# shibatch/rectdetect

Hardware: AMD Instinct MI355X
Metric: 1920x1080 frames/sec (higher is better)
Workload: dtype u8/i32/f32 (bit-exact integer + IEEE f32 stencil path)

## Files before the change

### rectdetect_amd/csrc/rd_k_front.hip

```cpp
#include <stdlib.h>
#include "rd_device.h"
#include "rd_kernels.h"
#include "rectdetect_hip.h"

#define RD_LUT_ATTR __device__
#include "rd_luts.h"

namespace {

using namespace rd;
using namespace rdpix;

struct P3 { float *p[3]; };
struct P3c { const float *p[3]; };
struct SrcZ { const uint8_t *p[RD_ZB_MAX]; };

inline int cdiv(int a, int b) { return (a + b - 1) / b; }
inline dim3 grid2(int iw, int ih) { return dim3(cdiv(iw, 64), cdiv(ih, 4)); }
const dim3 block2(64, 4);
inline int grid1(int n) { int g = cdiv(n, 256); return g < 1 ? 1 : g; }

__device__ __forceinline__ int lerp_lut(const unsigned short *t, int c) { return t[c >> 8] * (256 - (c & 255)) + t[(c >> 8) + 1] * (c & 255); }

__device__ __forceinline__ uint32_t plab_of(const unsigned short *s_s2l, const unsigned short *s_cf, const unsigned short *s_cf2, int b, int g, int r) {
// ... 218 lines not shown
    int pb, pg, pr;
    if (!is_yuv(FMT)) {
      const int i = 4 * RW * sr + rdpix::bpp(FMT) * sx, c[3] = { byte(i), byte(i + 1), byte(i + 2) };
      pb = c[rb_swapped(FMT) ? 2 : 0]; pg = c[1]; pr = c[rb_swapped(FMT) ? 0 : 2];
    } else if (FMT == RD_PIX_NV12) yuv_bgr(byte(8 * sr + sx), byte(16 + 2 * j), byte(17 + 2 * j), pb, pg, pr);
    else yuv_bgr(byte(8 * sr + sx), byte(16 + j), byte(20 + j), pb, pg, pr);
    b += pb; g += pg; r += pr;
  }
  b >>= 2; g >>= 2; r >>= 2;
}

template <int FMT>
__global__ __launch_bounds__(256) void k_pix2plab_half_t(uint32_t *__restrict__ out, P3 dst, PixZ src, int iw, int ih, size_t zs) {
  const int z = blockIdx.z;
  const uint8_t *__restrict__ p0 = src.p[0][z], *__restrict__ p1 = src.p[1][z], *__restrict__ p2 = src.p[2][z];
  RD_ZSHIFT(zs, out, dst.p[0], dst.p[1], dst.p[2]);
  __shared__ unsigned short s_s2l[RD_LUT_S2L_N], s_cf[RD_LUT_CF_N], s_cf2[RD_LUT_CF_N];
  __shared__ unsigned short tile[3][64][66];
  const int tid = rd_ty() * 64 + threadIdx.x;
  const int x0 = blockIdx.x * 64, y0 = blockIdx.y * 64;
  const int cx = (tid & 15) * 4, r0 = tid >> 4;
  const int x = x0 + cx, m = min(iw - x, 4);
  uint32_t w[4][HalfW<FMT>::n] = {};
#pragma unroll
  for (int k = 0; k < 4; k++) {
    const int y = y0 + r0 + 16 * k;
    if (m > 0 && y < ih) pix_load_half<FMT>(w[k], p0, p1, p2, src.pitch, x, y, m, src.wide != 0);
  }
  for (int i = tid; i < RD_LUT_S2L_N; i += 256) s_s2l[i] = rd_lut_s2l[i];
  for (int i = tid; i < RD_LUT_CF_N; i += 256) { s_cf[i] = rd_lut_cfunc[i]; s_cf2[i] = rd_lut_cfunc2[i]; }
  __syncthreads();
#pragma unroll
  for (int k = 0; k < 4; k++) {
    const int r = r0 + 16 * k, y = y0 + r;
    if (m <= 0 || y >= ih) continue;
    uint32_t v[4];
#pragma unroll
    for (int j = 0; j < 4; j++) {
      int b, g, rr;
      pix_bgr_half<FMT>(w[k], j, b, g, rr);
      v[j] = plab_of(s_s2l, s_cf, s_cf2, b, g, rr);
      tile[0][r][cx + j] = (unsigned short)(v[j] & 4095u); tile[1][r][cx + j] = (unsigned short)((v[j] >> 12) & 1023u); tile[2][r][cx + j] = (unsigned short)((v[j] >> 22) & 1023u);
    }
    uint32_t *o = out + (size_t)y * iw + x;
    if (m == 4 && (iw & 3) == 0) *(uint4 *)o = make_uint4(v[0], v[1], v[2], v[3]);
    else for (int j = 0; j < m; j++) o[j] = v[j];
  }
  __syncthreads();
  for (int r = rd_ty(); r < 64; r += 4) {
    const int ox = y0 + threadIdx.x, oy = x0 + r;
    if (ox < ih && oy < iw)
      for (int k = 0; k < 3; k++) ((unsigned short *)dst.p[k])[(size_t)oy * ih + ox] = tile[k][threadIdx.x][r];
  }
}

template <typename LD, typename ST> __device__ __forceinline__ void ew4(int n, LD ld, ST st) {
  const int stride = gridDim.x * blockDim.x;
  int i = blockIdx.x * blockDim.x + threadIdx.x;
  for (; i + 3 * stride < n; i += 4 * stride) {
    const auto v0 = ld(i), v1 = ld(i + stride), v2 = ld(i + 2 * stride), v3 = ld(i + 3 * stride);
    st(i, v0); st(i + stride, v1); st(i + 2 * stride, v2); st(i + 3 * stride, v3);
  }
  for (; i < n; i += stride) st(i, ld(i));
}

__global__ void k_unpack_plab(float *__restrict__ L, float *__restrict__ a, float *__restrict__ b, const uint32_t *__restrict__ in, int n) {
  for (int i = blockIdx.x * blockDim.x + threadIdx.x; i < n; i += gridDim.x * blockDim.x) {
    float l, aa, bb;
    unpack_lab(in[i], l, aa, bb);
    L[i] = l; a[i] = aa; b[i] = bb;
  }
}

__global__ void k_pack_plab(uint32_t *__restrict__ out, const float *__restrict__ L, const float *__restrict__ a, const float *__restrict__ b, int n) {
  ew4(n, [=](int i) { return make_float3(L[i], a[i], b[i]); }, [=](int i, float3 v) { out[i] = pack_lab(v.x, v.y, v.z); });
}

template <int MODE>
__global__ __launch_bounds__(256) void k_transpose(P3 dst, P3c src, P3c fwd, P3c bwd, const uint32_t *__restrict__ plab, int np, int W, int H, const int *only_if) {
  if (only_if && *only_if == 0) return;
  __shared__ float tile[3][64][65];
  const int x0 = blockIdx.x * 64, y0 = blockIdx.y * 64;
  for (int r = rd_ty(); r < 64; r += 4) {
    const int x = x0 + threadIdx.x, y = y0 + r;
    if (x < W && y < H) {
      const size_t i = (size_t)y * W + x;
      if (MODE == 1) {
        float l, a, b;
        unpack_lab(plab[i], l, a, b);
        tile[0][r][threadIdx.x] = l; tile[1][r][threadIdx.x] = a; tile[2][r][threadIdx.x] = b;
      } else if (MODE == 2) {
        for (int k = 0; k < np; k++) tile[k][r][threadIdx.x] = bwd.p[k][i] + fwd.p[k][i] - src.p[k][i] * 0.3989422804f;
      } else {
        for (int k = 0; k < np; k++) tile[k][r][threadIdx.x] = src.p[k][i];
      }
    }
  }
  __syncthreads();
  for (int r = rd_ty(); r < 64; r += 4) {
    const int ox = y0 + threadIdx.x, oy = x0 + r;
    if (ox < H && oy < W)
      for (int k = 0; k < np; k++) dst.p[k][(size_t)oy * H + ox] = tile[k][threadIdx.x][r];
  }
}

#define IIR_C0 0.3989422804f
#define IIR_C1 0.1414542400f
#define IIR_C2 -0.0030406818f
#define IIR_C3 -0.0041116157f
#define IIR_C4 0.0006696623f
#define IIR_C5 0.0000498707f
#define IIR_C6 -0.0000449761f
#define IIR_C7 -0.0000051528f
#define IIR_C8 0.2519574622f
#define IIR_C9 -0.0098627835f
#define IIR_C10 -0.0067013653f
#define IIR_C11 0.0012572396f
#define IIR_C12 0.0000481394f
#define IIR_C13 -0.0000097781f
#define IIR_C14 0.0000006462f
#define IIR_WARM 11
#ifndef IIR_CH
#define IIR_CH 16
#endif

#define IF_ROWS_MIN 64
#define IF_WU 32
#define IF_PITCH 65
__host__ __device__ inline int if_nchunks(int H, int rows) {
  int n = (H + rows - 1) / rows;
  if (n > 1 && H % rows != 0 && H % rows < 8) n--;
  return n;
}

typedef float iir_f2 __attribute__((ext_vector_type(2)));
#define IIR_STATE iir_f2 q1 = 0, q2 = 0, q3 = 0, q4 = 0, q5 = 0, q6 = 0, q7 = 0
#define IIR_STEP(i0v)                                                                                                  \
  iir_f2 acc = (iir_f2){IIR_C1, IIR_C8} * q1;                                                                          \
  acc = acc + (iir_f2){IIR_C2, IIR_C9} * q2;                                                                           \
  acc = acc + (iir_f2){IIR_C3, IIR_C10} * q3;                                                                          \
  acc = acc + (iir_f2){IIR_C4, IIR_C11} * q4;                                                                          \
  acc = acc + (iir_f2){IIR_C5, IIR_C12} * q5;                                                                          \
  acc = acc + (iir_f2){IIR_C6, IIR_C13} * q6;                                                                          \
  acc = acc + (iir_f2){IIR_C7, IIR_C14} * q7;                                                                          \
  float d = (i0v) * IIR_C0;                                                                                            \
  d += acc.x;                                                                                                          \
  d += acc.y;
#define IIR_SHIFT(i0v)                                                                                                 \
  q7 = q6; q6 = q5; q5 = q4; q4 = q3; q3 = q2; q2 = q1; q1 = (iir_f2){(i0v), d};

template <int SRC16> struct iir_src { typedef float T; };
template <> struct iir_src<1> { typedef unsigned short T; };
template <int SRC16, typename T> __device__ __forceinline__ float iir_field(T v, float sc, float hf) {
  if (SRC16) return (float)(int)v * sc + hf;
  return (float)v;
}
template <int TOUT, int IF_ROWS, int SRC16>
__global__ __launch_bounds__(128) void k_iir_fused_edge(P3 dst, P3c src, float *__restrict__ tails, int W, int H, int nchunks, int nf, int *bad, int np, size_t zs) {
  __shared__ float fwt[(IF_ROWS + 8) * IF_PITCH];
  const int lane = threadIdx.x & 63, anti = threadIdx.x >> 6;
  const int k = blockIdx.y % np, c = nf + (int)blockIdx.z;
  float *dk = k == 0 ? dst.p[0] : (k == 1 ? dst.p[1] : dst.p[2]);
  const float *sk = k == 0 ? src.p[0] : (k == 1 ? src.p[1] : src.p[2]);
  { const size_t rd_zoff_ = (size_t)(blockIdx.y / np) * zs; RD_ZS1(dk); RD_ZS1(sk); RD_ZS1(tails); RD_ZS1(bad); }
  if (blockIdx.x == 0 && k == 0 && c == 0 && threadIdx.x == 0) *bad = 0;
  const int x = blockIdx.x * 64 + lane;
  const bool xin = x < W;
  typedef typename iir_src<SRC16>::T TS;
  const TS *__restrict__ in = (const TS *)sk;
  const unsigned xs = (unsigned)(xin ? x : W - 1) * (unsigned)sizeof(TS), x4 = (unsigned)(xin ? x : W - 1) * 4u;
#define IIR_ROW(ptr) (*(const TS *)((const char *)(ptr) + xs))
#define IIR_OUT(ptr) (*(float *)((char *)(ptr) + x4))
  const float sc = k == 0 ? 1.0f / 4096 : 1.0f / 1024, hf = k == 0 ? 0.5f / 4096 : 0.5f / 1024;
#define IIR_LD(v) iir_field<SRC16>(v, sc, hf)
  const int s0 = c * IF_ROWS, s1 = (c == nchunks - 1) ? H : s0 + IF_ROWS;
  const int mid = s0 + (s1 - s0) / 2;
  float *__restrict__ tl = tails + ((size_t)(k * nchunks + c) * 4 * 7) * W;
  const int ylo = -IIR_WARM, yhi = H + IIR_WARM;
  float cur[IIR_CH], nxt[IIR_CH];
  {
    IIR_STATE;
    if (!anti) {
      const int fb = (s0 - IF_WU <= ylo) ? ylo : s0 - IF_WU;
      const int total = s1 - fb;
#pragma unroll
      for (int j = 0; j < IIR_CH; j++) cur[j] = IIR_LD(IIR_ROW(in + (size_t)mirror1(clampi(fb + j, ylo, yhi), H) * W));
      for (int base = 0; base < total; base += IIR_CH) {
#pragma unroll
        for (int j = 0; j < IIR_CH; j++) nxt[j] = IIR_LD(IIR_ROW(in + (size_t)mirror1(clampi(fb + base + IIR_CH + j, ylo, yhi), H) * W));
#pragma unroll
        for (int j = 0; j < IIR_CH; j++) {
          const int yy = fb + base + j;
          if (yy == mid) __syncthreads();
          IIR_STEP(cur[j]);
          if (yy >= s0 && yy < mid) fwt[(yy - s0) * IF_PITCH + lane] = d;
          else if (yy >= mid && yy < s1) {
            const float o = (fwt[(yy - s0) * IF_PITCH + lane] + d) - cur[j] * IIR_C0;
            if (TOUT) fwt[(yy - s0) * IF_PITCH + lane] = o;
            else if (xin) IIR_OUT(dk + (size_t)yy * W) = o;
          }
          if (xin && yy >= s0 - 7 && yy < s0) IIR_OUT(tl + (size_t)(0 * 7 + yy - (s0 - 7)) * W) = d;
          if (xin && yy >= s1 - 7 && yy < s1) IIR_OUT(tl + (size_t)(1 * 7 + yy - (s1 - 7)) * W) = d;
          IIR_SHIFT(cur[j]);
        }
#pragma unroll
        for (int j = 0; j < IIR_CH; j++) cur[j] = nxt[j];
      }
    } else {
      const int bb = (s1 - 1 + IF_WU >= yhi) ? yhi : s1 - 1 + IF_WU;
      const int total = bb - s0 + 1;
#pragma unroll
      for (int j = 0; j < IIR_CH; j++) cur[j] = IIR_LD(IIR_ROW(in + (size_t)mirror1(clampi(bb - j, ylo, yhi), H) * W));
      for (int base = 0; base < total; base += IIR_CH) {
#pragma unroll
        for (int j = 0; j < IIR_CH; j++) nxt[j] = IIR_LD(IIR_ROW(in + (size_t)mirror1(clampi(bb - (base + IIR_CH + j), ylo, yhi), H) * W));
#pragma unroll
        for (int j = 0; j < IIR_CH; j++) {
          const int yy = bb - (base + j);
          if (yy == mid - 1) __syncthreads();
          IIR_STEP(cur[j]);
          if (yy >= mid && yy < s1) fwt[(yy - s0) * IF_PITCH + lane] = d;
          else if (yy >= s0 && yy < mid) {
            const float o = d + fwt[(yy - s0) * IF_PITCH + lane] - cur[j] * IIR_C0;
            if (TOUT) fwt[(yy - s0) * IF_PITCH + lane] = o;
            else if (xin) IIR_OUT(dk + (size_t)yy * W) = o;
          }
          if (xin && yy >= s1 && yy < s1 + 7) IIR_OUT(tl + (size_t)(2 * 7 + yy - s1) * W) = d;
          if (xin && yy >= s0 && yy < s0 + 7) IIR_OUT(tl + (size_t)(3 * 7 + yy - s0) * W) = d;
          IIR_SHIFT(cur[j]);
        }
#pragma unroll
        for (int j = 0; j < IIR_CH; j++) cur[j] = nxt[j];
      }
    }
  }
  if (TOUT) {
    __syncthreads();
    const int rows = s1 - s0;
    for (int col = anti; col < 64; col += 2) {
      const int xx = blockIdx.x * 64 + col;
      if (xx >= W) break;
      float *__restrict__ o = dk + (size_t)xx * H + s0;
      for (int r = lane; r < rows; r += 64) at32(o, (unsigned)r) = fwt[r * IF_PITCH + col];
    }
  }
}

__device__ __forceinline__ unsigned iir_off(unsigned o) { asm("" : "+v"(o)); return o; }
template <typename T> __device__ __forceinline__ __attribute__((address_space(1))) T *iir_uni(T *p) {
  __attribute__((address_space(1))) T *g = (__attribute__((address_space(1))) T *)p;
  asm("" : "+s"(g));
  return g;
}
#ifndef IIR_PCH
#define IIR_PCH 16
#endif
#ifndef IF_TB
#define IF_TB 32
#endif
#define IF_TP (64 + 64 / IF_TB)
#ifdef IF_WPE
#define IF_WPE_ATTR __attribute__((amdgpu_waves_per_eu(IF_WPE)))
#else
#define IF_WPE_ATTR
#endif
template <int TOUT, int IF_ROWS, int SRC16>
__global__ __launch_bounds__(128) IF_WPE_ATTR void k_iir_fused(P3 dst, P3c src, float *__restrict__ tails, int W, int H, int nchunks, int *bad, int np, size_t zs) {
  constexpr int HALF = IF_ROWS / 2, CH = IIR_PCH, CPI = 64 / IF_TB;
  static_assert(CH >= 8 && IF_WU % CH == 0 && HALF % CH == 0 && HALF % IF_TB == 0 && 64 % IF_TB == 0, "whole chunks and whole batches, half a block per phase");
  __shared__ float swp[2 * 14 * 64];
  __shared__ float stg[TOUT ? 2 * IF_TB * IF_TP : 1];
  const int lane = threadIdx.x & 63, anti = __builtin_amdgcn_readfirstlane((int)(threadIdx.x >> 6));
  const int fz = __builtin_amdgcn_readfirstlane((int)(blockIdx.y / np)), k = blockIdx.y - fz * np, c = blockIdx.z;
  float *dk = k == 0 ? dst.p[0] : (k == 1 ? dst.p[1] : dst.p[2]);
  const float *sk = k == 0 ? src.p[0] : (k == 1 ? src.p[1] : src.p[2]);
  { const size_t rd_zoff_ = (size_t)fz * zs; RD_ZS1(dk); RD_ZS1(sk); RD_ZS1(tails); RD_ZS1(bad); }
  if (blockIdx.x == 0 && k == 0 && blockIdx.z == 0 && threadIdx.x == 0) *bad = 0;
  const int x = blockIdx.x * 64 + lane;
  const bool xin = x < W;
  typedef typename iir_src<SRC16>::T TS;
  const TS *__restrict__ in = (const TS *)sk;
  const unsigned xs = (unsigned)(xin ? x : W - 1) * (unsigned)sizeof(TS), x4 = (unsigned)(xin ? x : W - 1) * 4u;
#undef IIR_ROW
#undef IIR_OUT
#define IIR_ROW(ptr) (*(const TS *)((const char *)(ptr) + xo_))
#define IIR_OUT(ptr) (*(float *)((char *)(ptr) + iir_off(x4)))
  const float sc = k == 0 ? 1.0f / 4096 : 1.0f / 1024, hf = k == 0 ? 0.5f / 4096 : 0.5f / 1024;
  const int s0 = c * IF_ROWS, s1 = s0 + IF_ROWS, mid = s0 + HALF;
  float *__restrict__ tl = tails + ((size_t)(k * nchunks + c) * 4 * 7) * W;
  const long rs = anti ? -(long)W : (long)W;
  float cur[CH], nxt[CH], park[HALF];
#define IIR_PSTEPS(...)                                                                                                  \
      _Pragma("unroll") for (int j = 0; j < CH; j++) {                                                                   \
        IIR_STEP(cur[j]);                                                                                                \
        __VA_ARGS__;                                                                                                     \
        IIR_SHIFT(cur[j]);                                                                                               \
      }                                                                                                                  \
      _Pragma("unroll") for (int j = 0; j < CH; j++) cur[j] = nxt[j];
#define IIR_PCHUNK(MORE, NEXT, NSTEP, ...)                                                                               \
    {                                                                                                                    \
      if (MORE) { const TS *n_ = (NEXT); const unsigned xo_ = iir_off(xs); _Pragma("unroll") for (int j = 0; j < CH; j++) { nxt[j] = IIR_LD(IIR_ROW(iir_uni(n_))); n_ += (NSTEP); } } \
      IIR_PSTEPS(__VA_ARGS__)                                                                                            \
    }
#define IIR_PARK(dst, v) asm("v_mov_b32 %0, %1" : "=v"(dst) : "v"(v))
  IIR_STATE;
  const TS *p = in + (size_t)(anti ? s1 - 1 : s0) * W;
  const TS *const pb = in + (size_t)(anti ? mid : mid - 1) * W;
  float *const tw = tl + (size_t)(anti ? 2 * 7 + 6 : 0) * W;
#define IIR_WTAIL if (j >= CH - 7 && xin) IIR_OUT(iir_uni(tw + (long)(j - (CH - 7)) * rs)) = d
  if (anti ? s1 + IF_WU <= H : s0 - IF_WU >= 0) {
    const TS *w = p - IF_WU * rs;
    { const unsigned xo_ = iir_off(xs);
#pragma unroll
      for (int j = 0; j < CH; j++) cur[j] = IIR_LD(IIR_ROW(iir_uni(w + (long)j * rs))); }
    for (int q = 0; q < IF_WU / CH - 1; q++) { IIR_PCHUNK(1, w + CH * rs, rs, (void)0); w += CH * rs; }
    IIR_PCHUNK(1, p, rs, IIR_WTAIL);
  } else {
    const int dy = anti ? -1 : 1, y0 = anti ? s1 - 1 + IF_WU : s0 - IF_WU;
    const unsigned xo_ = iir_off(xs);
    auto eld = [&](int yy) -> float {
      const int yc = clampi(yy, -IIR_WARM, H + IIR_WARM);
      const float v = IIR_LD(IIR_ROW(iir_uni(in + (size_t)mirror1(yc, H) * W)));
      return yy == yc ? v : 0.0f;
    };
#define IIR_PCHUNK_E(YN, ...) { _Pragma("unroll") for (int j = 0; j < CH; j++) nxt[j] = eld((YN) + j * dy); IIR_PSTEPS(__VA_ARGS__) }
#pragma unroll
    for (int j = 0; j < CH; j++) cur[j] = eld(y0 + j * dy);
    for (int q = 0; q < IF_WU / CH - 1; q++) IIR_PCHUNK_E(y0 + (q + 1) * CH * dy, (void)0)
    IIR_PCHUNK(1, p, rs, IIR_WTAIL);
  }
#undef IIR_WTAIL
#pragma unroll
  for (int q = 0; q < HALF / CH; q++) {
    const bool last = q == HALF / CH - 1;
    IIR_PCHUNK(1, last ? pb : p + CH * rs, last ? -rs : rs, IIR_PARK(park[q * CH + j], d)); p += CH * rs;
  }
  {
    float *mine = swp + anti * (14 * 64) + lane, *theirs = swp + (anti ^ 1) * (14 * 64) + lane;
#define IIR_SWAP(n, q) mine[(2 * n) * 64] = q.x; mine[(2 * n + 1) * 64] = q.y;
    IIR_SWAP(0, q1) IIR_SWAP(1, q2) IIR_SWAP(2, q3) IIR_SWAP(3, q4) IIR_SWAP(4, q5) IIR_SWAP(5, q6) IIR_SWAP(6, q7)
#undef IIR_SWAP
    __syncthreads();
#define IIR_SWAP(n, q) q.x = theirs[(2 * n) * 64]; q.y = theirs[(2 * n + 1) * 64];
    IIR_SWAP(0, q1) IIR_SWAP(1, q2) IIR_SWAP(2, q3) IIR_SWAP(3, q4) IIR_SWAP(4, q5) IIR_SWAP(5, q6) IIR_SWAP(6, q7)
#undef IIR_SWAP
  }
  p = pb;
  float *const tt = tl + (size_t)(anti ? 1 * 7 : 3 * 7 + 6) * W;
  float *o = dk + (size_t)(anti ? mid : mid - 1) * W;
  float *const st = stg + (TOUT ? anti * (IF_TB * IF_TP) : 0);
  const int br = lane % IF_TB, bc = lane / IF_TB;
  const float *const sl = st + (anti ? br : IF_TB - 1 - br) * IF_TP + bc;
  const unsigned bo = ((unsigned)bc * (unsigned)H + (unsigned)br) * 4u;
#pragma unroll
  for (int q = 0; q < HALF / CH; q++) {
    const bool last = q == HALF / CH - 1;
    IIR_PCHUNK(!last, p - CH * rs, -rs, {
      const int i = q * CH + j;
      const float r = (park[HALF - 1 - i] + d) - cur[j] * IIR_C0;
      if (TOUT) st[(i % IF_TB) * IF_TP + lane] = r; else if (xin) IIR_OUT(iir_uni(o - (long)j * rs)) = r;
      if (i >= HALF - 7 && xin) IIR_OUT(iir_uni(tt - (long)(i - (HALF - 7)) * rs)) = d;
      if (TOUT && i % IF_TB == IF_TB - 1) {
        __builtin_amdgcn_fence(__ATOMIC_RELEASE, "wavefront"); __builtin_amdgcn_wave_barrier(); __builtin_amdgcn_fence(__ATOMIC_ACQUIRE, "wavefront");
        const int lowest = anti ? mid + (i / IF_TB) * IF_TB : mid - (i / IF_TB + 1) * IF_TB;
        float *const ob = dk + (size_t)(blockIdx.x * 64) * H + lowest;
        _Pragma("unroll") for (int n = 0; n < IF_TB; n++)
          if ((int)blockIdx.x * 64 + n * CPI + bc < W) *(float *)((char *)iir_uni(ob + (size_t)(n * CPI) * H) + bo) = sl[n * CPI];
        __builtin_amdgcn_fence(__ATOMIC_RELEASE, "wavefront"); __builtin_amdgcn_wave_barrier(); __builtin_amdgcn_fence(__ATOMIC_ACQUIRE, "wavefront");
      }
    });
    p -= CH * rs; if (!TOUT) o -= CH * rs;
  }
#undef IIR_PCHUNK
#undef IIR_PCHUNK_E
#undef IIR_PSTEPS
#undef IIR_PARK
}

#undef IIR_LD
#undef IIR_ROW
#undef IIR_OUT

#define IC_CH 4
template <int TOUT, int SRC16, int EAGER>
__global__ __launch_bounds__(64 * IC_CH) void k_iir_check_fix(P3 dst, P3c src, P3 fwd, const float *__restrict__ tails, int *bad, int W, int H, int nchunks, int IF_ROWS, int force, int np, size_t zs) {
  const int x = blockIdx.x * 64 + threadIdx.x;
  const int k = blockIdx.y % np, c = blockIdx.z * IC_CH + rd_ty();
  if (c >= nchunks) return;
  float *dk = k == 0 ? dst.p[0] : (k == 1 ? dst.p[1] : dst.p[2]), *fk = k == 0 ? fwd.p[0] : (k == 1 ? fwd.p[1] : fwd.p[2]);
  const float *sk = k == 0 ? src.p[0] : (k == 1 ? src.p[1] : src.p[2]);
  { const size_t rd_zoff_ = (size_t)(blockIdx.y / np) * zs; RD_ZS1(dk); RD_ZS1(sk); RD_ZS1(fk); RD_ZS1(tails); RD_ZS1(bad); }
  if (x >= W) return;
  const int s0 = c * IF_ROWS, s1 = (c == nchunks - 1) ? H : s0 + IF_ROWS;
  const float *me = tails + ((size_t)(k * nchunks + c) * 4 * 7) * W + x;
  bool differ = force != 0 && c == 0;
  const bool chk_f = c > 0 && s0 - IF_WU > -IIR_WARM;
  const bool chk_b = c < nchunks - 1 && s1 - 1 + IF_WU < H + IIR_WARM;
  const float *pv = tails + ((size_t)(k * nchunks + (chk_f ? c - 1 : c)) * 4 * 7) * W + x;
  const float *nx = tails + ((size_t)(k * nchunks + (chk_b ? c + 1 : c)) * 4 * 7) * W + x;
  if (EAGER) {
    unsigned a[14], b[14];
#pragma unroll
    for (int j = 0; j < 7; j++) {
      a[j] = __float_as_uint(me[(size_t)(0 * 7 + j) * W]); b[j] = __float_as_uint(pv[(size_t)(1 * 7 + j) * W]);
      a[7 + j] = __float_as_uint(me[(size_t)(2 * 7 + j) * W]); b[7 + j] = __float_as_uint(nx[(size_t)(3 * 7 + j) * W]);
    }
    unsigned df = 0, db = 0;
#pragma unroll
    for (int j = 0; j < 7; j++) { df |= a[j] ^ b[j]; db |= a[7 + j] ^ b[7 + j]; }
    differ = differ || (chk_f && df != 0) || (chk_b && db != 0);
  } else {
    if (chk_f) {
#pragma unroll
      for (int j = 0; j < 7; j++) differ = differ || (__float_as_uint(me[(size_t)(0 * 7 + j) * W]) != __float_as_uint(pv[(size_t)(1 * 7 + j) * W]));
    }
    if (chk_b) {
#pragma unroll
      for (int j = 0; j < 7; j++) differ = differ || (__float_as_uint(me[(size_t)(2 * 7 + j) * W]) != __float_as_uint(nx[(size_t)(3 * 7 + j) * W]));
    }
  }
  if (!differ) return;
  atomicOr(bad, 1);
  typedef typename iir_src<SRC16>::T TS;
  const TS *__restrict__ in = (const TS *)sk + x;
  const float sc = k == 0 ? 1.0f / 4096 : 1.0f / 1024, hf = k == 0 ? 0.5f / 4096 : 0.5f / 1024;
  float *fw = fk + x;
  {
    IIR_STATE;
    for (int yy = -IIR_WARM; yy < H; yy++) {
      const float i0 = iir_field<SRC16>(in[(size_t)mirror1(yy, H) * W], sc, hf);
      IIR_STEP(i0);
      if (yy >= 0) fw[(size_t)yy * W] = d;
      IIR_SHIFT(i0);
    }
  }
  {
    IIR_STATE;
    for (int yy = H + IIR_WARM; yy >= 0; yy--) {
      const float i0 = iir_field<SRC16>(in[(size_t)mirror1(yy, H) * W], sc, hf);
      IIR_STEP(i0);
      if (yy < H) {
        const float o = d + fw[(size_t)yy * W] - i0 * IIR_C0;
        if (TOUT) dk[(size_t)x * H + yy] = o; else dk[(size_t)yy * W + x] = o;
      }
      IIR_SHIFT(i0);
    }
  }
}

#define RD_IIRCOEF_ATTR __device__ __constant__
#include "rd_iircoef.h"
__global__ __launch_bounds__(128) void k_iir_line(float *dst, const float *__restrict__ src, float *fw, float *bw, int W, int H, int r) {
  const int x = blockIdx.x * 64 + threadIdx.x;
  const bool xin = x < W;
  float C[15];
#pragma unroll
  for (int k = 0; k < 15; k++) C[k] = rd_iircoef[r][k];
  const int warm = r + 1 + 8;
  if (xin) {
    const float *in = src + x;
    float i1 = 0, i2 = 0, i3 = 0, i4 = 0, i5 = 0, i6 = 0, i7 = 0;
    float t0 = 0, t1 = 0, t2 = 0, t3 = 0, t4 = 0, t5 = 0, t6 = 0;
#define IIR_LINE_STEP                                                                                                    \
    const float i0 = in[(size_t)mirror1(yy, H) * W];                                                                     \
    float d = i0 * C[0];                                                                                                 \
    d += C[1] * i1 + C[2] * i2 + C[3] * i3 + C[4] * i4 + C[5] * i5 + C[6] * i6 + C[7] * i7;                              \
    d += C[8] * t0 + C[9] * t1 + C[10] * t2 + C[11] * t3 + C[12] * t4 + C[13] * t5 + C[14] * t6;                         \
    i7 = i6; i6 = i5; i5 = i4; i4 = i3; i3 = i2; i2 = i1; i1 = i0;                                                       \
    t6 = t5; t5 = t4; t4 = t3; t3 = t2; t2 = t1; t1 = t0; t0 = d;
    if (rd_ty() == 0) {
      float *o = fw + x;
      for (int yy = -warm; yy < H; yy++) { IIR_LINE_STEP; if (yy >= 0) o[(size_t)yy * W] = d; }
    } else {
      float *o = bw + x;
      for (int yy = H + warm; yy >= 0; yy--) { IIR_LINE_STEP; if (yy < H) o[(size_t)yy * W] = d; }
    }
#undef IIR_LINE_STEP
  }
  __syncthreads();
  if (!xin) return;
  for (int yy = rd_ty(); yy < H; yy += 2) {
    const size_t p = (size_t)yy * W + x;
    dst[p] = bw[p] + fw[p] - src[p] * C[0];
  }
}

#include "rd_front_helpers.h"

#ifndef EV_PX
#define EV_PX 4
#endif
__device__ __forceinline__ void ev_finish(float2 *__restrict__ dst, int p, float vx, float vy) {
  float len = vx * vx + vy * vy;
  if ((double)len > 1e-10) {
    len = 1.0f / sqrtf(len);
    vx *= len; vy *= len;
  } else {
    vx = vy = 0.70710678118f;
  }
  dst[p] = make_float2(vx, vy);
}
__global__ __launch_bounds__(256) void k_edgevec(float2 *__restrict__ dst, const float *__restrict__ in, int iw, int ih, uint32_t *__restrict__ pack_out, const float *__restrict__ pa, const float *__restrict__ pb, size_t zs) {
  RD_ZSHIFT(zs, dst, in, pack_out, pa, pb);
  const int x = blockIdx.x * 64 + threadIdx.x, y0 = (blockIdx.y * 4 + rd_ty()) * EV_PX;
  if (x >= iw || y0 >= ih) return;
  if (pack_out != nullptr) {
#pragma unroll
    for (int k = 0; k < EV_PX; k++) if (y0 + k < ih) { const int p = (y0 + k) * iw + x; pack_out[p] = pack_lab(in[p], pa[p], pb[p]); }
  }
  const bool interior = blockIdx.x > 0 && blockIdx.y > 0 && (int)(blockIdx.x * 64 + 66) <= iw && (int)((blockIdx.y * 4 + 4) * EV_PX + 2) <= ih;
  if (interior) {
    float w[EV_PX + 4][5];
#pragma unroll
    for (int r = 0; r < EV_PX + 4; r++) {
      const float *row = in + (size_t)(y0 + r - 2) * iw + x;
#pragma unroll
      for (int c = 0; c < 5; c++) w[r][c] = row[c - 2];
    }
#pragma unroll
    for (int k = 0; k < EV_PX; k++) {
      float vx = 0, vy = 0;
#pragma unroll
      for (int yy = -2; yy <= 2; yy++)
#pragma unroll
        for (int xx = -2; xx <= 2; xx++) {
          const float s = w[k + yy + 2][xx + 2];
          vx += v5c((xx + 2) + (yy + 2) * 5) * s;
          vy += v5c((yy + 2) + (xx + 2) * 5) * s;
        }
// ... 166 lines not shown
  const int x = blockIdx.x * 64 + threadIdx.x, y = blockIdx.y * 4 + rd_ty();
  if (x >= iw || y >= ih) return;
  const int c = in[y * iw + x];
  uint8_t *o = out + (size_t)y * ws + x * 3;
  if (c == bgc) { o[0] = 0; o[1] = 0; o[2] = 0; return; }
  const int g = (int)((unsigned)c * 1103515245u + 12345u);
  o[2] = (uint8_t)((((g & (7 << 0)) << 5) | 31) & 255);
  o[1] = (uint8_t)((((g & (7 << 3)) << 2) | 31) & 255);
  o[0] = (uint8_t)((((g & (7 << 6)) >> 1) | 31) & 255);
}

__device__ __forceinline__ float icfunc(float ft) { return ft > 0.20689270648f ? ft * ft * ft : (ft - 16.0f / 116) * (1.0f / 7.787f); }

__global__ __launch_bounds__(256) void k_plab2bgr(uint8_t *__restrict__ out, const uint32_t *__restrict__ in, int iw, int ih, int ws) {
  const int x = blockIdx.x * 64 + threadIdx.x, y = blockIdx.y * 4 + rd_ty();
  if (x >= iw || y >= ih) return;
  const float xn = 0.950456f, zn = 1.088754f;
  float L, a, b;
  unpack_lab(in[y * iw + x], L, a, b);
  L *= 256; a *= 256; b *= 256;
  float cy;
  if (L > 0.20689270648f) { cy = (L + 16) * (1.0f / 116.0f); cy = cy * cy * cy; }
  else cy = L * (1.0f / 903.3f);
  const float fy = (float)(rd_lut_cfunc[clampi((int)floorf(cy * 1024), 0, 1023)] + 9039) * (1.0f / 65536.0f);
  const float fz = fy - (b - 128) * (1.0f / 200.0f);
  const float fx = fy + (a - 128) * (1.0f / 500.0f);
  const float cx = icfunc(fx) * xn, cz = icfunc(fz) * zn;
  const float r = cx * 3.240479f + cy * -1.537150f + cz * -0.498535f;
  const float g = cx * -0.969256f + cy * 1.875991f + cz * 0.041556f;
  const float bb = cx * 0.055648f + cy * -0.204043f + cz * 1.057311f;
  uint8_t *o = out + (size_t)y * ws + x * 3;
  o[2] = rd_lut_l2s[clampi((int)floorf(r * 1024), 0, 1023)];
  o[1] = rd_lut_l2s[clampi((int)floorf(g * 1024), 0, 1023)];
  o[0] = rd_lut_l2s[clampi((int)floorf(bb * 1024), 0, 1023)];
}

__global__ __launch_bounds__(256) void k_edge_f(float *__restrict__ out, const float *__restrict__ in, int iw, int ih) {
  const int x = blockIdx.x * 64 + threadIdx.x, y = blockIdx.y * 4 + rd_ty();
  if (x >= iw || y >= ih) return;
  const float n = in[mirror2(x, y - 1, iw, ih)], s = in[mirror2(x, y + 1, iw, ih)], w = in[mirror2(x - 1, y, iw, ih)], e = in[mirror2(x + 1, y, iw, ih)];
  float sum = 0, t;
  t = n + w - s - e;
  sum += (in[mirror2(x - 1, y - 1, iw, ih)] - in[mirror2(x + 1, y + 1, iw, ih)]) * t;
  t = n - w + e - s;
  sum += (in[mirror2(x + 1, y - 1, iw, ih)] - in[mirror2(x - 1, y + 1, iw, ih)]) * t;
  out[y * iw + x] = sqrtf(fmaxf(0.0f, sum));
}

__global__ __launch_bounds__(256) void k_edgevec_plab(float2 *__restrict__ dst, const uint32_t *__restrict__ in, int iw, int ih) {
  const int x = blockIdx.x * 64 + threadIdx.x, y = blockIdx.y * 4 + rd_ty();
  if (x >= iw || y >= ih) return;
  float vx3[3] = { 0, 0, 0 }, vy3[3] = { 0, 0, 0 };
#pragma unroll
  for (int yy = -2; yy <= 2; yy++) {
#pragma unroll
    for (int xx = -2; xx <= 2; xx++) {
      float s[3];
      unpack_lab(in[mirror2(x + xx, y + yy, iw, ih)], s[0], s[1], s[2]);
#pragma unroll
      for (int c = 0; c < 3; c++) {
        vx3[c] += v5c((xx + 2) + (yy + 2) * 5) * s[c];
        vy3[c] += v5c((yy + 2) + (xx + 2) * 5) * s[c];
      }
    }
  }
  float l3[3];
#pragma unroll
  for (int c = 0; c < 3; c++) l3[c] = vx3[c] * vx3[c] + vy3[c] * vy3[c];
  float ivlen, vx, vy;
  if (l3[0] >= l3[1] && l3[0] >= l3[2]) { ivlen = l3[0]; vx = vx3[0]; vy = vy3[0]; }
  else if (l3[1] >= l3[2]) { ivlen = l3[1]; vx = vx3[1]; vy = vy3[1]; }
  else { ivlen = l3[2]; vx = vx3[2]; vy = vy3[2]; }
  if ((double)l3[0] >= 1e-6 && (vx3[0] * vx + vy3[0] * vy < 0)) { vx = -vx; vy = -vy; }
  if ((double)ivlen > 1e-10) { ivlen = 1.0f / sqrtf(ivlen); vx *= ivlen; vy *= ivlen; }
  else vx = vy = 0.70710678118f;
  dst[y * iw + x] = make_float2(vx, vy);
}

__global__ __launch_bounds__(256) void k_thincubic(float *__restrict__ out, const float *__restrict__ in, const float2 *__restrict__ vxy, int iw, int ih) {
  const int x = blockIdx.x * 64 + threadIdx.x, y = blockIdx.y * 4 + rd_ty();
  if (x >= iw || y >= ih) return;
  const int p0 = y * iw + x;
  const float2 v = vxy[p0];
  const float am2 = bicubic(in, x - 2 * v.x, y - 2 * v.y, iw, ih);
  const float am1 = bicubic(in, x - 1 * v.x, y - 1 * v.y, iw, ih);
  const float a0 = in[p0];
  const float ap1 = bicubic(in, x + 1 * v.x, y + 1 * v.y, iw, ih);
  const float ap2 = bicubic(in, x + 2 * v.x, y + 2 * v.y, iw, ih);
  const float C = 0.99f;
  out[p0] = (am2 * C <= a0 && am1 * C <= a0 && a0 >= ap1 * C && a0 >= ap2 * C) ? (am2 + am1 + a0 + ap1 + ap2) : 0.0f;
}

}

namespace rdk {

void bgr2plab(hipStream_t s, uint32_t *out, const uint8_t *bgr, int iw, int ih, int ws) {
  hipLaunchKernelGGL(k_bgr2plab, dim3(cdiv(iw, 64), cdiv(ih, 16)), block2, 0, s, out, bgr, iw, ih, ws);
}
void bgr2plab_transposed(hipStream_t s, uint32_t *out, float *const dst[3], const uint8_t *const *bgr, int iw, int ih, int ws, int nz, size_t zs) {
  P3 d = { { dst[0], dst[1], dst[2] } };
  SrcZ z;
  for (int i = 0; i < RD_ZB_MAX; i++) z.p[i] = bgr[i < nz ? i : 0];
  hipLaunchKernelGGL(k_bgr2plab_t, dim3(cdiv(iw, 64), cdiv(ih, 64), nz), block2, 0, s, out, d, z, iw, ih, ws, zs);
}
void bgr2plab_transposed(hipStream_t s, uint32_t *out, float *const dst[3], const uint8_t *bgr, int iw, int ih, int ws) {
  bgr2plab_transposed(s, out, dst, &bgr, iw, ih, ws, 1, 0);
}
static PixZ pixz_of(const uint8_t *const (*planes)[3], const int pitch[3], int nz) {
  PixZ z;
  z.wide = 1;
  for (int k = 0; k < 3; k++) {
    z.pitch[k] = pitch[k];
    if (pitch[k] & 3) z.wide = 0;
    for (int i = 0; i < RD_ZB_MAX; i++) { z.p[k][i] = planes[i < nz ? i : 0][k]; if ((uintptr_t)z.p[k][i] & 3) z.wide = 0; }
  }
  return z;
}
void pix2plab_transposed(hipStream_t s, int fmt, uint32_t *out, float *const dst[3], const uint8_t *const (*planes)[3], const int pitch[3], int iw, int ih, int nz, size_t zs) {
  const P3 d = { { dst[0], dst[1], dst[2] } };
  const PixZ z = pixz_of(planes, pitch, nz);
  const dim3 grid(cdiv(iw, 64), cdiv(ih, 64), nz);
  const bool known = fmt != RD_PIX_BGR && dispatch(fmt, [&](auto f) {
    if constexpr (f.value != RD_PIX_BGR) hipLaunchKernelGGL(k_pix2plab_t<f.value>, grid, block2, 0, s, out, d, z, iw, ih, zs);
  });
  if (!known) abort();
}
void pix2plab_half_transposed(hipStream_t s, int fmt, uint32_t *out, float *const dst[3], const uint8_t *const (*planes)[3], const int pitch[3], int iw, int ih, int nz, size_t zs) {
  const P3 d = { { dst[0], dst[1], dst[2] } };
  const PixZ z = pixz_of(planes, pitch, nz);
  const dim3 grid(cdiv(iw, 64), cdiv(ih, 64), nz);
  if (!dispatch(fmt, [&](auto f) { hipLaunchKernelGGL(k_pix2plab_half_t<f.value>, grid, block2, 0, s, out, d, z, iw, ih, zs); })) abort();
}
void unpack_plab(hipStream_t s, float *L, float *a, float *b, const uint32_t *in, int n) {
  hipLaunchKernelGGL(k_unpack_plab, dim3(ew_grid(n)), dim3(256), 0, s, L, a, b, in, n);
}
void pack_plab(hipStream_t s, uint32_t *out, const float *L, const float *a, const float *b, int n) {
  hipLaunchKernelGGL(k_pack_plab, dim3(ew_grid(n)), dim3(256), 0, s, out, L, a, b, n);
}

static P3 mk3(float *const p[3], int np) { P3 r = { { nullptr, nullptr, nullptr } }; for (int k = 0; k < np; k++) r.p[k] = p[k]; return r; }
static P3c mk3c(const float *const p[3], int np) { P3c r = { { nullptr, nullptr, nullptr } }; for (int k = 0; k < np; k++) r.p[k] = p[k]; return r; }

void transpose_f(hipStream_t s, float *const dst[3], const float *const src[3], int np, int W, int H) {
  P3c z = { { nullptr, nullptr, nullptr } };
  hipLaunchKernelGGL(k_transpose<0>, dim3(cdiv(W, 64), cdiv(H, 64)), block2, 0, s, mk3(dst, np), mk3c(src, np), z, z, (const uint32_t *)nullptr, np, W, H, (const int *)nullptr);
}
static int if_pick_rows(int np, int W, int H, int transpose_out, int nz) {
  (void)np; (void)W; (void)H;
  (void)transpose_out;
#ifndef IF_GROUP_ROWS
#define IF_GROUP_ROWS 128
#endif
  if (nz > 1) return IF_GROUP_ROWS;
  return 64;
}

size_t iir_pass_scratch_floats(int np, int W, int H) { return (size_t)np * if_nchunks(H, IF_ROWS_MIN) * 4 * 7 * W; }

void iir_blur_pass(hipStream_t s, float *const dst[3], const float *const src[3], float *const fwd[3], float *const bwd[3], int np, int W, int H,
                   int transpose_out, float *tails, int *bad, int src16, int nz, size_t zs) {
  const int rows = if_pick_rows(np, W, H, transpose_out, nz);
  const int nchunks = if_nchunks(H, rows);
  const int nf = (H - (nchunks - 1) * rows == rows) ? nchunks : nchunks - 1;
  const dim3 grid(cdiv(W, 64), np * nz, nchunks);
  const dim3 fgrid(grid.x, grid.y, nf), egrid(grid.x, grid.y, nchunks - nf);
#define IF_LAUNCH(T, R, S16) { if (nf > 0) hipLaunchKernelGGL((k_iir_fused<T, R, S16>), fgrid, dim3(128), 0, s, mk3(dst, np), mk3c(src, np), tails, W, H, nchunks, bad, np, zs); \
    if (nf < nchunks) hipLaunchKernelGGL((k_iir_fused_edge<T, R, S16>), egrid, dim3(128), 0, s, mk3(dst, np), mk3c(src, np), tails, W, H, nchunks, nf, bad, np, zs); }
#define IF_LAUNCH_R(R) { if (transpose_out && src16) IF_LAUNCH(1, R, 1) else if (transpose_out) IF_LAUNCH(1, R, 0) else IF_LAUNCH(0, R, 0) }
  switch (rows) {
    case 64: IF_LAUNCH_R(64); break;
#if IF_GROUP_ROWS != 64 && IF_GROUP_ROWS != 128
    case IF_GROUP_ROWS: IF_LAUNCH_R(IF_GROUP_ROWS); break;
#endif
    default: IF_LAUNCH_R(128); break;
  }
#undef IF_LAUNCH_R
#undef IF_LAUNCH
  if (nchunks > 1) {
    const dim3 cgrid(grid.x, grid.y, cdiv(nchunks, IC_CH)), cblock(64, IC_CH);
    const int force = getenv("RD_IIR_FORCE_FIX") ? 1 : 0;
#define IC_LAUNCH(T, S16, E) hipLaunchKernelGGL((k_iir_check_fix<T, S16, E>), cgrid, cblock, 0, s, mk3(dst, np), mk3c(src, np), mk3(fwd, np), (const float *)tails, bad, W, H, nchunks, rows, force, np, zs)
    if (nz > 1) { if (transpose_out && src16) IC_LAUNCH(1, 1, 0); else if (transpose_out) IC_LAUNCH(1, 0, 0); else IC_LAUNCH(0, 0, 0); }
    else { if (transpose_out && src16) IC_LAUNCH(1, 1, 1); else if (transpose_out) IC_LAUNCH(1, 0, 1); else IC_LAUNCH(0, 0, 1); }
#undef IC_LAUNCH
  }
  (void)bwd;
}

void iir_blur_lines(hipStream_t s, float *dst, const float *src, float *fw, float *bw, int W, int H, int r) {
  hipLaunchKernelGGL(k_iir_line, dim3(cdiv(W, 64)), dim3(64, 2), 0, s, dst, src, fw, bw, W, H, r);
}

void convert_bgr_lumaf(hipStream_t s, uint8_t *out, const float *in, float f, int iw, int ih, int ws) {
  hipLaunchKernelGGL(k_convert_bgr_lumaf, grid2(iw, ih), block2, 0, s, out, in, f, iw, ih, ws);
}
void convert_bgr_labeli(hipStream_t s, uint8_t *out, const int *in, int bgc, int iw, int ih, int ws) {
  hipLaunchKernelGGL(k_convert_bgr_labeli, grid2(iw, ih), block2, 0, s, out, in, bgc, iw, ih, ws);
}
void plab2bgr(hipStream_t s, uint8_t *out, const uint32_t *in, int iw, int ih, int ws) {
  hipLaunchKernelGGL(k_plab2bgr, grid2(iw, ih), block2, 0, s, out, in, iw, ih, ws);
}
void edge_f(hipStream_t s, float *out, const float *in, int iw, int ih) {
  hipLaunchKernelGGL(k_edge_f, grid2(iw, ih), block2, 0, s, out, in, iw, ih);
}
void edgevec_plab(hipStream_t s, float *vxy, const uint32_t *in, int iw, int ih) {
  hipLaunchKernelGGL(k_edgevec_plab, grid2(iw, ih), block2, 0, s, (float2 *)vxy, in, iw, ih);
}
void thincubic(hipStream_t s, float *out, const float *in, const float *vxy, int iw, int ih) {
  hipLaunchKernelGGL(k_thincubic, grid2(iw, ih), block2, 0, s, out, in, (const float2 *)vxy, iw, ih);
}
void edgevec(hipStream_t s, float *vxy, const float *in, int iw, int ih, uint32_t *pack_out, const float *a, const float *b, int nz, size_t zs) {
  hipLaunchKernelGGL(k_edgevec, dim3(cdiv(iw, 64), cdiv(ih, 4 * EV_PX), nz), block2, 0, s, (float2 *)vxy, in, iw, ih, pack_out, a, b, zs);
}
void edge_plab(hipStream_t s, float *out, const uint32_t *in, int iw, int ih, int nz, size_t zs) {
  hipLaunchKernelGGL(k_edge_plab, dim3(cdiv(iw, 64), cdiv(ih, 4 * EP_PX), nz), block2, 0, s, out, in, iw, ih, zs);
}
void thinthres(hipStream_t s, float *out, const float *in, const float *vxy, int iw, int ih, int nz, size_t zs) {
  hipLaunchKernelGGL(k_thinthres, dim3(cdiv(iw, 64), cdiv(ih, TT_ROWS), nz), dim3(64, 4), 0, s, out, in, (const float2 *)vxy, iw, ih, zs);
}
void threshold_f(hipStream_t s, float *out, const float *in, float lo, float thr, float hi, int n) {
  hipLaunchKernelGGL(k_threshold_f, dim3(ew_grid(n)), dim3(256), 0, s, out, in, lo, thr, hi, n);
}
void threshold_i(hipStream_t s, int *out, const int *in, int lo, int thr, int hi, int n) {
  hipLaunchKernelGGL(k_threshold_i, dim3(ew_grid(n)), dim3(256), 0, s, out, in, lo, thr, hi, n);
}
void cast_i_f(hipStream_t s, int *out, const float *in, float scale, int n) {
  hipLaunchKernelGGL(k_cast_i_f, dim3(ew_grid(n)), dim3(256), 0, s, out, in, scale, n);
}
void cast_c_i(hipStream_t s, int8_t *out, const int *in, int n) {
  hipLaunchKernelGGL(k_cast_c_i, dim3(ew_grid(n)), dim3(256), 0, s, out, in, n);
}
void clear_i(hipStream_t s, int *out, int n) {
  if (n > 0) hipLaunchKernelGGL(k_clear_i, dim3(ew_grid(n)), dim3(256), 0, s, out, n);
}
void copy_i(hipStream_t s, int *out, const int *in, int n) {
  if (n > 0) hipLaunchKernelGGL(k_copy_i, dim3(ew_grid(n)), dim3(256), 0, s, out, in, n);
}
void rand_i(hipStream_t s, int *out, uint64_t seed, int n) {
  if (n > 0) hipLaunchKernelGGL(k_rand_i, dim3(ew_grid(n)), dim3(256), 0, s, out, seed, n);
}

}
```

Baseline: 3494.

## Handle partial last IIR chunk in fused kernel by shifting window, park in LDS

The last, partial row-chunk is now handled inside the fast fused IIR kernel. Its window is shifted to end at H, and outputs and tail states are written only for the rows that chunk owns, so the slower edge kernel no longer runs for it. For large non-transposed chunks, part of the backward-pass park buffer is moved from registers into LDS to reduce register pressure. Smaller tweaks add an fmaf in the u16 field conversion, an unguarded transpose-store path for full-width blocks, and an optional row-size override. The price is extra per-step trigger checks and a second template instantiation, which enlarge the code.

```diff
diff --git a/rectdetect_amd/csrc/rd_k_front.hip b/rectdetect_amd/csrc/rd_k_front.hip
--- a/rectdetect_amd/csrc/rd_k_front.hip
+++ b/rectdetect_amd/csrc/rd_k_front.hip
@@ -394,7 +394,7 @@
 template <int SRC16> struct iir_src { typedef float T; };
 template <> struct iir_src<1> { typedef unsigned short T; };
 template <int SRC16, typename T> __device__ __forceinline__ float iir_field(T v, float sc, float hf) {
-  if (SRC16) return (float)(int)v * sc + hf;
+  if (SRC16) return __builtin_fmaf((float)(int)v, sc, hf);
   return (float)v;
 }
 template <int TOUT, int IF_ROWS, int SRC16>
@@ -497,6 +497,9 @@
 #ifndef IIR_PCH
 #define IIR_PCH 16
 #endif
+#ifndef IF_LPARK
+#define IF_LPARK 24
+#endif
 #ifndef IF_TB
 #define IF_TB 32
 #endif
@@ -506,12 +509,11 @@
 #else
 #define IF_WPE_ATTR
 #endif
-template <int TOUT, int IF_ROWS, int SRC16>
-__global__ __launch_bounds__(128) IF_WPE_ATTR void k_iir_fused(P3 dst, P3c src, float *__restrict__ tails, int W, int H, int nchunks, int *bad, int np, size_t zs) {
-  constexpr int HALF = IF_ROWS / 2, CH = IIR_PCH, CPI = 64 / IF_TB;
-  static_assert(CH >= 8 && IF_WU % CH == 0 && HALF % CH == 0 && HALF % IF_TB == 0 && 64 % IF_TB == 0, "whole chunks and whole batches, half a block per phase");
-  __shared__ float swp[2 * 14 * 64];
-  __shared__ float stg[TOUT ? 2 * IF_TB * IF_TP : 1];
+template <int TOUT, int IF_ROWS, int SRC16, int MOVED>
+__device__ __forceinline__ void iir_fused_block(P3 dst, P3c src, float *__restrict__ tails, int W, int H, int nchunks, int *bad, int np, size_t zs, float *swp, float *stg, float *lpk) {
+  constexpr int HALF = IF_ROWS / 2, CH = (MOVED && IF_ROWS <= 64) ? 8 : IIR_PCH, CPI = 64 / IF_TB;
+  constexpr int LP = (!TOUT && IF_ROWS > 64) ? IF_LPARK : 0;
+  static_assert(CH >= 8 && IF_WU % CH == 0 && HALF % CH == 0 && (!TOUT || HALF % IF_TB == 0) && 64 % IF_TB == 0 && HALF <= 64 && LP < HALF, "whole chunks and whole batches, half a block per phase");
   const int lane = threadIdx.x & 63, anti = __builtin_amdgcn_readfirstlane((int)(threadIdx.x >> 6));
   const int fz = __builtin_amdgcn_readfirstlane((int)(blockIdx.y / np)), k = blockIdx.y - fz * np, c = blockIdx.z;
   float *dk = k == 0 ? dst.p[0] : (k == 1 ? dst.p[1] : dst.p[2]);
@@ -528,35 +530,46 @@
 #define IIR_ROW(ptr) (*(const TS *)((const char *)(ptr) + xo_))
 #define IIR_OUT(ptr) (*(float *)((char *)(ptr) + iir_off(x4)))
   const float sc = k == 0 ? 1.0f / 4096 : 1.0f / 1024, hf = k == 0 ? 0.5f / 4096 : 0.5f / 1024;
-  const int s0 = c * IF_ROWS, s1 = s0 + IF_ROWS, mid = s0 + HALF;
+  const int lim = c * IF_ROWS, s0 = MOVED ? H - IF_ROWS : lim, s1 = s0 + IF_ROWS, mid = s0 + HALF, skip = lim - s0;
   float *__restrict__ tl = tails + ((size_t)(k * nchunks + c) * 4 * 7) * W;
   const long rs = anti ? -(long)W : (long)W;
-  float cur[CH], nxt[CH], park[HALF];
-#define IIR_PSTEPS(...)                                                                                                  \
+  const int trig1 = anti ? IF_ROWS - skip : skip, trig2 = anti ? skip - HALF : HALF - skip;
+#define IIR_T1(n) (MOVED && (n) == trig1)
+#define IIR_T2(n) (MOVED && (n) == trig2)
+#define IIR_DUMP(base, stp) if (xin) { float *const b_ = (base); const long s_ = (stp);                                  \
+    IIR_OUT(iir_uni(b_)) = q1.y; IIR_OUT(iir_uni(b_ + s_)) = q2.y; IIR_OUT(iir_uni(b_ + 2 * s_)) = q3.y; IIR_OUT(iir_uni(b_ + 3 * s_)) = q4.y;                       \
+    IIR_OUT(iir_uni(b_ + 4 * s_)) = q5.y; IIR_OUT(iir_uni(b_ + 5 * s_)) = q6.y; IIR_OUT(iir_uni(b_ + 6 * s_)) = q7.y; }
+  float *const d1 = tl + (size_t)(anti ? 3 * 7 : 6) * W, *const d2 = tl + (size_t)(anti ? 6 : 3 * 7) * W;
+  const int tc = trig2 < 0 ? 0 : (trig2 > HALF ? HALF : trig2);
+  const unsigned long long below = tc >= 64 ? ~0ull : (1ull << tc) - 1ull, smask = anti ? ~below : below;
+  float cur[CH], nxt[CH], park[HALF - LP];
+  float *const lp = lpk + anti * (LP * 64) + lane;
+#define IIR_PSTEPS(PRE, ...)                                                                                             \
       _Pragma("unroll") for (int j = 0; j < CH; j++) {                                                                   \
+        PRE;                                                                                                             \
         IIR_STEP(cur[j]);                                                                                                \
         __VA_ARGS__;                                                                                                     \
         IIR_SHIFT(cur[j]);                                                                                               \
       }                                                                                                                  \
       _Pragma("unroll") for (int j = 0; j < CH; j++) cur[j] = nxt[j];
-#define IIR_PCHUNK(MORE, NEXT, NSTEP, ...)                                                                               \
+#define IIR_PCHUNK(MORE, NEXT, NSTEP, PRE, ...)                                                                           \
     {                                                                                                                    \
       if (MORE) { const TS *n_ = (NEXT); const unsigned xo_ = iir_off(xs); _Pragma("unroll") for (int j = 0; j < CH; j++) { nxt[j] = IIR_LD(IIR_ROW(iir_uni(n_))); n_ += (NSTEP); } } \
-      IIR_PSTEPS(__VA_ARGS__)                                                                                            \
-    }
-#define IIR_PARK(dst, v) asm("v_mov_b32 %0, %1" : "=v"(dst) : "v"(v))
+      IIR_PSTEPS(PRE, __VA_ARGS__)                                                                                       \
+    }
+#define IIR_PARK(n, v) { if ((n) < LP) lp[(n) * 64] = (v); else asm("v_mov_b32 %0, %1" : "=v"(park[(n) < LP ? 0 : (n) - LP]) : "v"(v)); }
   IIR_STATE;
   const TS *p = in + (size_t)(anti ? s1 - 1 : s0) * W;
   const TS *const pb = in + (size_t)(anti ? mid : mid - 1) * W;
   float *const tw = tl + (size_t)(anti ? 2 * 7 + 6 : 0) * W;
-#define IIR_WTAIL if (j >= CH - 7 && xin) IIR_OUT(iir_uni(tw + (long)(j - (CH - 7)) * rs)) = d
+#define IIR_WTAIL if (!MOVED && j >= CH - 7 && xin) IIR_OUT(iir_uni(tw + (long)(j - (CH - 7)) * rs)) = d
   if (anti ? s1 + IF_WU <= H : s0 - IF_WU >= 0) {
     const TS *w = p - IF_WU * rs;
     { const unsigned xo_ = iir_off(xs);
 #pragma unroll
       for (int j = 0; j < CH; j++) cur[j] = IIR_LD(IIR_ROW(iir_uni(w + (long)j * rs))); }
-    for (int q = 0; q < IF_WU / CH - 1; q++) { IIR_PCHUNK(1, w + CH * rs, rs, (void)0); w += CH * rs; }
-    IIR_PCHUNK(1, p, rs, IIR_WTAIL);
+    for (int q = 0; q < IF_WU / CH - 1; q++) { IIR_PCHUNK(1, w + CH * rs, rs, (void)0, (void)0); w += CH * rs; }
+    IIR_PCHUNK(1, p, rs, (void)0, IIR_WTAIL);
   } else {
     const int dy = anti ? -1 : 1, y0 = anti ? s1 - 1 + IF_WU : s0 - IF_WU;
     const unsigned xo_ = iir_off(xs);
@@ -565,18 +578,20 @@
       const float v = IIR_LD(IIR_ROW(iir_uni(in + (size_t)mirror1(yc, H) * W)));
       return yy == yc ? v : 0.0f;
     };
-#define IIR_PCHUNK_E(YN, ...) { _Pragma("unroll") for (int j = 0; j < CH; j++) nxt[j] = eld((YN) + j * dy); IIR_PSTEPS(__VA_ARGS__) }
+#define IIR_PCHUNK_E(YN) { _Pragma("unroll") for (int j = 0; j < CH; j++) nxt[j] = eld((YN) + j * dy); IIR_PSTEPS((void)0, (void)0) }
 #pragma unroll
     for (int j = 0; j < CH; j++) cur[j] = eld(y0 + j * dy);
-    for (int q = 0; q < IF_WU / CH - 1; q++) IIR_PCHUNK_E(y0 + (q + 1) * CH * dy, (void)0)
-    IIR_PCHUNK(1, p, rs, IIR_WTAIL);
+    for (int q = 0; q < IF_WU / CH - 1; q++) IIR_PCHUNK_E(y0 + (q + 1) * CH * dy)
+    IIR_PCHUNK(1, p, rs, (void)0, IIR_WTAIL);
   }
 #undef IIR_WTAIL
+  if (MOVED && anti) IIR_DUMP(tl + (size_t)(2 * 7) * W, (long)W)
 #pragma unroll
   for (int q = 0; q < HALF / CH; q++) {
     const bool last = q == HALF / CH - 1;
-    IIR_PCHUNK(1, last ? pb : p + CH * rs, last ? -rs : rs, IIR_PARK(park[q * CH + j], d)); p += CH * rs;
-  }
+    IIR_PCHUNK(1, last ? pb : p + CH * rs, last ? -rs : rs, if (IIR_T1(q * CH + j)) IIR_DUMP(d1, -rs), IIR_PARK(q * CH + j, d)); p += CH * rs;
+  }
+  if (IIR_T1(HALF)) IIR_DUMP(d1, -rs)
   {
     float *mine = swp + anti * (14 * 64) + lane, *theirs = swp + (anti ^ 1) * (14 * 64) + lane;
 #define IIR_SWAP(n, q) mine[(2 * n) * 64] = q.x; mine[(2 * n + 1) * 64] = q.y;
@@ -597,26 +612,46 @@
 #pragma unroll
   for (int q = 0; q < HALF / CH; q++) {
     const bool last = q == HALF / CH - 1;
-    IIR_PCHUNK(!last, p - CH * rs, -rs, {
+    IIR_PCHUNK(!last, p - CH * rs, -rs, if (IIR_T2(q * CH + j)) IIR_DUMP(d2, rs), {
       const int i = q * CH + j;
-      const float r = (park[HALF - 1 - i] + d) - cur[j] * IIR_C0;
-      if (TOUT) st[(i % IF_TB) * IF_TP + lane] = r; else if (xin) IIR_OUT(iir_uni(o - (long)j * rs)) = r;
-      if (i >= HALF - 7 && xin) IIR_OUT(iir_uni(tt - (long)(i - (HALF - 7)) * rs)) = d;
+      float pk;
+      if (HALF - 1 - i < LP) pk = lp[(HALF - 1 - i) * 64]; else pk = park[HALF - 1 - i < LP ? 0 : HALF - 1 - i - LP];
+      const float r = (pk + d) - cur[j] * IIR_C0;
+      if (TOUT) st[(i % IF_TB) * IF_TP + lane] = r; else if (xin && (!MOVED || ((smask >> i) & 1))) IIR_OUT(iir_uni(o - (long)j * rs)) = r;
+      if (!MOVED && i >= HALF - 7 && xin) IIR_OUT(iir_uni(tt - (long)(i - (HALF - 7)) * rs)) = d;
       if (TOUT && i % IF_TB == IF_TB - 1) {
         __builtin_amdgcn_fence(__ATOMIC_RELEASE, "wavefront"); __builtin_amdgcn_wave_barrier(); __builtin_amdgcn_fence(__ATOMIC_ACQUIRE, "wavefront");
         const int lowest = anti ? mid + (i / IF_TB) * IF_TB : mid - (i / IF_TB + 1) * IF_TB;
         float *const ob = dk + (size_t)(blockIdx.x * 64) * H + lowest;
-        _Pragma("unroll") for (int n = 0; n < IF_TB; n++)
-          if ((int)blockIdx.x * 64 + n * CPI + bc < W) *(float *)((char *)iir_uni(ob + (size_t)(n * CPI) * H) + bo) = sl[n * CPI];
+        const int cb = (!MOVED || lowest + br >= lim) ? (int)blockIdx.x * 64 + bc : 0x3fffffff;
+        if (!MOVED && SRC16 && (int)blockIdx.x * 64 + 64 <= W) {
+          _Pragma("unroll") for (int n = 0; n < IF_TB; n++) *(float *)((char *)iir_uni(ob + (size_t)(n * CPI) * H) + bo) = sl[n * CPI];
+        } else {
+          _Pragma("unroll") for (int n = 0; n < IF_TB; n++)
+            if (cb + n * CPI < W) *(float *)((char *)iir_uni(ob + (size_t)(n * CPI) * H) + bo) = sl[n * CPI];
+        }
         __builtin_amdgcn_fence(__ATOMIC_RELEASE, "wavefront"); __builtin_amdgcn_wave_barrier(); __builtin_amdgcn_fence(__ATOMIC_ACQUIRE, "wavefront");
       }
     });
     p -= CH * rs; if (!TOUT) o -= CH * rs;
   }
+  if (MOVED && anti) IIR_DUMP(tl + (size_t)(1 * 7 + 6) * W, -(long)W)
+#undef IIR_DUMP
+#undef IIR_T1
+#undef IIR_T2
 #undef IIR_PCHUNK
 #undef IIR_PCHUNK_E
 #undef IIR_PSTEPS
 #undef IIR_PARK
+}
+template <int TOUT, int IF_ROWS, int SRC16>
+__global__ __launch_bounds__(128) IF_WPE_ATTR void k_iir_fused(P3 dst, P3c src, float *__restrict__ tails, int W, int H, int nchunks, int *bad, int np, size_t zs) {
+  constexpr int LP = (!TOUT && IF_ROWS > 64) ? IF_LPARK : 0;
+  __shared__ float swp[2 * 14 * 64];
+  __shared__ float stg[TOUT ? 2 * IF_TB * IF_TP : 1];
+  __shared__ float lpk[LP ? 2 * LP * 64 : 1];
+  if (((int)blockIdx.z + 1) * IF_ROWS <= H) iir_fused_block<TOUT, IF_ROWS, SRC16, 0>(dst, src, tails, W, H, nchunks, bad, np, zs, swp, stg, lpk);
+  else iir_fused_block<TOUT, IF_ROWS, SRC16, 1>(dst, src, tails, W, H, nchunks, bad, np, zs, swp, stg, lpk);
 }
 
 #undef IIR_LD
@@ -1089,6 +1124,9 @@
 #ifndef IF_GROUP_ROWS
 #define IF_GROUP_ROWS 128
 #endif
+#ifdef IF_GROUP_ROWS_Y
+  if (nz > 1 && !transpose_out) return IF_GROUP_ROWS_Y;
+#endif
   if (nz > 1) return IF_GROUP_ROWS;
   return 64;
 }
@@ -1099,7 +1137,8 @@
                    int transpose_out, float *tails, int *bad, int src16, int nz, size_t zs) {
   const int rows = if_pick_rows(np, W, H, transpose_out, nz);
   const int nchunks = if_nchunks(H, rows);
-  const int nf = (H - (nchunks - 1) * rows == rows) ? nchunks : nchunks - 1;
+  const int lastrows = H - (nchunks - 1) * rows;
+  const int nf = (lastrows == rows || (nchunks > 1 && lastrows < rows)) ? nchunks : nchunks - 1;
   const dim3 grid(cdiv(W, 64), np * nz, nchunks);
   const dim3 fgrid(grid.x, grid.y, nf), egrid(grid.x, grid.y, nchunks - nf);
 #define IF_LAUNCH(T, R, S16) { if (nf > 0) hipLaunchKernelGGL((k_iir_fused<T, R, S16>), fgrid, dim3(128), 0, s, mk3(dst, np), mk3c(src, np), tails, W, H, nchunks, bad, np, zs); \
@@ -1110,6 +1149,9 @@
 #if IF_GROUP_ROWS != 64 && IF_GROUP_ROWS != 128
     case IF_GROUP_ROWS: IF_LAUNCH_R(IF_GROUP_ROWS); break;
 #endif
+#ifdef IF_GROUP_ROWS_Y
+    case IF_GROUP_ROWS_Y: IF_LAUNCH(0, IF_GROUP_ROWS_Y, 0); break;
+#endif
     default: IF_LAUNCH_R(128); break;
   }
 #undef IF_LAUNCH_R
```

Result: no change. 3470 (-0.7%).
